# facebookresearch/fast3r

Hardware: NVIDIA H100
Metric: views_per_sec (higher is better)
Workload: dtype bf16

## Files before the change

fast3r_b200/csrc/common.cuh:

```cuda
#pragma once
#include <cuda.h>
#include <cuda_bf16.h>
#include <cuda_fp16.h>
#include <cuda_runtime.h>
#include <stdint.h>

#include <type_traits>

namespace f3r {

#define F3R_DEVICE __device__ __forceinline__

F3R_DEVICE uint32_t smem_u32(const void* p) { return static_cast<uint32_t>(__cvta_generic_to_shared(p)); }

F3R_DEVICE uint32_t lane_id() { return threadIdx.x & 31; }

F3R_DEVICE bool elect_one() {
  uint32_t pred = 0;
  asm volatile(
      "{\n\t.reg .pred P;\n\t"
      "elect.sync _|P, 0xffffffff;\n\t"
      "selp.u32 %0, 1, 0, P;\n\t}\n"
      : "=r"(pred));
  return pred != 0;
}

F3R_DEVICE void mbar_init(uint64_t* bar, uint32_t count) {
  asm volatile("mbarrier.init.shared::cta.b64 [%0], %1;" ::"r"(smem_u32(bar)), "r"(count));
}
F3R_DEVICE void fence_barrier_init() { asm volatile("fence.mbarrier_init.release.cluster;" ::: "memory"); }
F3R_DEVICE void fence_proxy_async_smem() { asm volatile("fence.proxy.async.shared::cta;" ::: "memory"); }

F3R_DEVICE void mbar_arrive(uint64_t* bar) {
  asm volatile("mbarrier.arrive.shared::cta.b64 _, [%0];" ::"r"(smem_u32(bar)) : "memory");
}
F3R_DEVICE void mbar_arrive_expect_tx(uint64_t* bar, uint32_t bytes) {
  asm volatile("mbarrier.arrive.expect_tx.shared::cta.b64 _, [%0], %1;" ::"r"(smem_u32(bar)), "r"(bytes) : "memory");
}
F3R_DEVICE bool mbar_try_wait(uint64_t* bar, uint32_t parity) {
  uint32_t ok;
  asm volatile(
      "{\n\t.reg .pred P;\n\t"
      "mbarrier.try_wait.parity.shared::cta.b64 P, [%1], %2;\n\t"
      "selp.u32 %0, 1, 0, P;\n\t}\n"
      : "=r"(ok)
      : "r"(smem_u32(bar)), "r"(parity)
      : "memory");
  return ok != 0;
}
F3R_DEVICE void mbar_wait(uint64_t* bar, uint32_t parity) {
  while (!mbar_try_wait(bar, parity)) {
  }
}

F3R_DEVICE void mbar_wait_relaxed(uint64_t* bar, uint32_t parity) {
  while (!mbar_try_wait(bar, parity)) asm volatile("nanosleep.u32 64;");
}

F3R_DEVICE void tma_prefetch_desc(const CUtensorMap* m) {
  asm volatile("prefetch.tensormap [%0];" ::"l"(reinterpret_cast<uint64_t>(m)) : "memory");
}
F3R_DEVICE void tma_load_2d(void* dst, const CUtensorMap* m, uint64_t* bar, int c0, int c1) {
  asm volatile(
      "cp.async.bulk.tensor.2d.shared::cluster.global.mbarrier::complete_tx::bytes [%0], [%1, {%3, %4}], [%2];"
      ::"r"(smem_u32(dst)), "l"(reinterpret_cast<uint64_t>(m)), "r"(smem_u32(bar)), "r"(c0), "r"(c1)
      : "memory");
}
F3R_DEVICE void tma_load_3d(void* dst, const CUtensorMap* m, uint64_t* bar, int c0, int c1, int c2) {
  asm volatile(
      "cp.async.bulk.tensor.3d.shared::cluster.global.mbarrier::complete_tx::bytes [%0], [%1, {%3, %4, %5}], [%2];"
      ::"r"(smem_u32(dst)), "l"(reinterpret_cast<uint64_t>(m)), "r"(smem_u32(bar)), "r"(c0), "r"(c1), "r"(c2)
      : "memory");
}
F3R_DEVICE void tma_load_4d(void* dst, const CUtensorMap* m, uint64_t* bar, int c0, int c1, int c2, int c3) {
  asm volatile(
      "cp.async.bulk.tensor.4d.shared::cluster.global.mbarrier::complete_tx::bytes [%0], [%1, {%3, %4, %5, %6}], [%2];"
      ::"r"(smem_u32(dst)), "l"(reinterpret_cast<uint64_t>(m)), "r"(smem_u32(bar)), "r"(c0), "r"(c1), "r"(c2),
      "r"(c3)
      : "memory");
}

F3R_DEVICE void tma_store_4d(const CUtensorMap* m, const void* src, int c0, int c1, int c2, int c3) {
  asm volatile("cp.async.bulk.tensor.4d.global.shared::cta.bulk_group [%0, {%2, %3, %4, %5}], [%1];"
               ::"l"(reinterpret_cast<uint64_t>(m)), "r"(smem_u32(src)), "r"(c0), "r"(c1), "r"(c2), "r"(c3)
               : "memory");
}
F3R_DEVICE void tma_reduce_add_4d(const CUtensorMap* m, const void* src, int c0, int c1, int c2, int c3) {
  asm volatile("cp.reduce.async.bulk.tensor.4d.global.shared::cta.add.tile.bulk_group [%0, {%2, %3, %4, %5}], [%1];"
               ::"l"(reinterpret_cast<uint64_t>(m)), "r"(smem_u32(src)), "r"(c0), "r"(c1), "r"(c2), "r"(c3)
               : "memory");
}
F3R_DEVICE void tma_store_commit() { asm volatile("cp.async.bulk.commit_group;" ::: "memory"); }
F3R_DEVICE void tma_store_wait_read() { asm volatile("cp.async.bulk.wait_group.read 0;" ::: "memory"); }
F3R_DEVICE void tma_store_wait_all() { asm volatile("cp.async.bulk.wait_group 0;" ::: "memory"); }

F3R_DEVICE void pdl_wait() { asm volatile("griddepcontrol.wait;" ::: "memory"); }
F3R_DEVICE void pdl_launch_dependents() { asm volatile("griddepcontrol.launch_dependents;" ::: "memory"); }

F3R_DEVICE uint32_t cluster_ctarank() { uint32_t r; asm volatile("mov.u32 %0, %%cluster_ctarank;" : "=r"(r)); return r; }
F3R_DEVICE uint32_t cluster_id_x() { uint32_t r; asm volatile("mov.u32 %0, %%clusterid.x;" : "=r"(r)); return r; }
F3R_DEVICE uint32_t num_clusters_x() { uint32_t r; asm volatile("mov.u32 %0, %%nclusterid.x;" : "=r"(r)); return r; }
F3R_DEVICE void cluster_sync_all() {
  asm volatile("barrier.cluster.arrive.release.aligned;" ::: "memory");
  asm volatile("barrier.cluster.wait.acquire.aligned;" ::: "memory");
}

F3R_DEVICE uint64_t make_smem_desc_sw128(uint32_t smem_addr) {
  uint64_t d = 0;
  d |= static_cast<uint64_t>((smem_addr & 0x3FFFF) >> 4);
  d |= static_cast<uint64_t>(1) << 16;
  d |= static_cast<uint64_t>(1024 >> 4) << 32;
  d |= static_cast<uint64_t>(1) << 62;
  return d;
}
F3R_DEVICE void wgmma_fence() { asm volatile("wgmma.fence.sync.aligned;" ::: "memory"); }
F3R_DEVICE void wgmma_commit() { asm volatile("wgmma.commit_group.sync.aligned;" ::: "memory"); }
template <int kPending>
F3R_DEVICE void wgmma_wait() { asm volatile("wgmma.wait_group.sync.aligned %0;" ::"n"(kPending) : "memory"); }
template <int kN>
F3R_DEVICE void fence_regs(float (&d)[kN]) {
#pragma unroll
  for (int i = 0; i < kN; ++i) asm volatile("" : "+f"(d[i])::"memory");
}


template <typename T>
constexpr bool is_f16 = std::is_same<T, __half>::value;

#define F3R_WGMMA_SS_N128(TY) \
  asm volatile( \
      "{\n\t.reg .pred p;\n\t" \
      "setp.ne.b32 p, %66, 0;\n\t" \
      "wgmma.mma_async.sync.aligned.m64n128k16.f32." TY "." TY " {%0, %1, %2, %3, %4, %5, %6, %7, %8, %9, %10, %11, %12, %13, %14, %15, %16, %17, %18, %19, %20, %21, %22, %23, %24, %25, %26, %27, %28, %29, %30, %31, %32, %33, %34, %35, %36, %37, %38, %39, %40, %41, %42, %43, %44, %45, %46, %47, %48, %49, %50, %51, %52, %53, %54, %55, %56, %57, %58, %59, %60, %61, %62, %63}, %64, %65, p, 1, 1, 0, %67;\n\t}\n" \
      : "+f"(d[0]), "+f"(d[1]), "+f"(d[2]), "+f"(d[3]), "+f"(d[4]), "+f"(d[5]), "+f"(d[6]), "+f"(d[7]), "+f"(d[8]), "+f"(d[9]), "+f"(d[10]), "+f"(d[11]), "+f"(d[12]), "+f"(d[13]), "+f"(d[14]), "+f"(d[15]), "+f"(d[16]), "+f"(d[17]), "+f"(d[18]), "+f"(d[19]), "+f"(d[20]), "+f"(d[21]), "+f"(d[22]), "+f"(d[23]), "+f"(d[24]), "+f"(d[25]), "+f"(d[26]), "+f"(d[27]), "+f"(d[28]), "+f"(d[29]), "+f"(d[30]), "+f"(d[31]), "+f"(d[32]), "+f"(d[33]), "+f"(d[34]), "+f"(d[35]), "+f"(d[36]), "+f"(d[37]), "+f"(d[38]), "+f"(d[39]), "+f"(d[40]), "+f"(d[41]), "+f"(d[42]), "+f"(d[43]), "+f"(d[44]), "+f"(d[45]), "+f"(d[46]), "+f"(d[47]), "+f"(d[48]), "+f"(d[49]), "+f"(d[50]), "+f"(d[51]), "+f"(d[52]), "+f"(d[53]), "+f"(d[54]), "+f"(d[55]), "+f"(d[56]), "+f"(d[57]), "+f"(d[58]), "+f"(d[59]), "+f"(d[60]), "+f"(d[61]), "+f"(d[62]), "+f"(d[63]) \
      : "l"(a_desc), "l"(b_desc), "r"(accumulate), "n"(kTransB))
template <int kTransB, typename T = __nv_bfloat16>
F3R_DEVICE void wgmma_ss_n128(float (&d)[64], uint64_t a_desc, uint64_t b_desc, uint32_t accumulate) {
  if constexpr (is_f16<T>) F3R_WGMMA_SS_N128("f16");
  else F3R_WGMMA_SS_N128("bf16");
}

#define F3R_WGMMA_SS_N256(TY) \
  asm volatile( \
      "{\n\t.reg .pred p;\n\t" \
      "setp.ne.b32 p, %130, 0;\n\t" \
      "wgmma.mma_async.sync.aligned.m64n256k16.f32." TY "." TY " {%0, %1, %2, %3, %4, %5, %6, %7, %8, %9, %10, %11, %12, %13, %14, %15, %16, %17, %18, %19, %20, %21, %22, %23, %24, %25, %26, %27, %28, %29, %30, %31, %32, %33, %34, %35, %36, %37, %38, %39, %40, %41, %42, %43, %44, %45, %46, %47, %48, %49, %50, %51, %52, %53, %54, %55, %56, %57, %58, %59, %60, %61, %62, %63, %64, %65, %66, %67, %68, %69, %70, %71, %72, %73, %74, %75, %76, %77, %78, %79, %80, %81, %82, %83, %84, %85, %86, %87, %88, %89, %90, %91, %92, %93, %94, %95, %96, %97, %98, %99, %100, %101, %102, %103, %104, %105, %106, %107, %108, %109, %110, %111, %112, %113, %114, %115, %116, %117, %118, %119, %120, %121, %122, %123, %124, %125, %126, %127}, %128, %129, p, 1, 1, 0, %131;\n\t}\n" \
      : "+f"(d[0]), "+f"(d[1]), "+f"(d[2]), "+f"(d[3]), "+f"(d[4]), "+f"(d[5]), "+f"(d[6]), "+f"(d[7]), "+f"(d[8]), "+f"(d[9]), "+f"(d[10]), "+f"(d[11]), "+f"(d[12]), "+f"(d[13]), "+f"(d[14]), "+f"(d[15]), "+f"(d[16]), "+f"(d[17]), "+f"(d[18]), "+f"(d[19]), "+f"(d[20]), "+f"(d[21]), "+f"(d[22]), "+f"(d[23]), "+f"(d[24]), "+f"(d[25]), "+f"(d[26]), "+f"(d[27]), "+f"(d[28]), "+f"(d[29]), "+f"(d[30]), "+f"(d[31]), "+f"(d[32]), "+f"(d[33]), "+f"(d[34]), "+f"(d[35]), "+f"(d[36]), "+f"(d[37]), "+f"(d[38]), "+f"(d[39]), "+f"(d[40]), "+f"(d[41]), "+f"(d[42]), "+f"(d[43]), "+f"(d[44]), "+f"(d[45]), "+f"(d[46]), "+f"(d[47]), "+f"(d[48]), "+f"(d[49]), "+f"(d[50]), "+f"(d[51]), "+f"(d[52]), "+f"(d[53]), "+f"(d[54]), "+f"(d[55]), "+f"(d[56]), "+f"(d[57]), "+f"(d[58]), "+f"(d[59]), "+f"(d[60]), "+f"(d[61]), "+f"(d[62]), "+f"(d[63]), "+f"(d[64]), "+f"(d[65]), "+f"(d[66]), "+f"(d[67]), "+f"(d[68]), "+f"(d[69]), "+f"(d[70]), "+f"(d[71]), "+f"(d[72]), "+f"(d[73]), "+f"(d[74]), "+f"(d[75]), "+f"(d[76]), "+f"(d[77]), "+f"(d[78]), "+f"(d[79]), "+f"(d[80]), "+f"(d[81]), "+f"(d[82]), "+f"(d[83]), "+f"(d[84]), "+f"(d[85]), "+f"(d[86]), "+f"(d[87]), "+f"(d[88]), "+f"(d[89]), "+f"(d[90]), "+f"(d[91]), "+f"(d[92]), "+f"(d[93]), "+f"(d[94]), "+f"(d[95]), "+f"(d[96]), "+f"(d[97]), "+f"(d[98]), "+f"(d[99]), "+f"(d[100]), "+f"(d[101]), "+f"(d[102]), "+f"(d[103]), "+f"(d[104]), "+f"(d[105]), "+f"(d[106]), "+f"(d[107]), "+f"(d[108]), "+f"(d[109]), "+f"(d[110]), "+f"(d[111]), "+f"(d[112]), "+f"(d[113]), "+f"(d[114]), "+f"(d[115]), "+f"(d[116]), "+f"(d[117]), "+f"(d[118]), "+f"(d[119]), "+f"(d[120]), "+f"(d[121]), "+f"(d[122]), "+f"(d[123]), "+f"(d[124]), "+f"(d[125]), "+f"(d[126]), "+f"(d[127]) \
      : "l"(a_desc), "l"(b_desc), "r"(accumulate), "n"(kTransB))
template <int kTransB, typename T = __nv_bfloat16>
F3R_DEVICE void wgmma_ss_n256(float (&d)[128], uint64_t a_desc, uint64_t b_desc, uint32_t accumulate) {
  if constexpr (is_f16<T>) F3R_WGMMA_SS_N256("f16");
  else F3R_WGMMA_SS_N256("bf16");
}

#define F3R_WGMMA_RS_N64(TY) \
  asm volatile( \
      "{\n\t.reg .pred p;\n\t" \
      "setp.ne.b32 p, %37, 0;\n\t" \
      "wgmma.mma_async.sync.aligned.m64n64k16.f32." TY "." TY " {%0, %1, %2, %3, %4, %5, %6, %7, %8, %9, %10, %11, %12, %13, %14, %15, %16, %17, %18, %19, %20, %21, %22, %23, %24, %25, %26, %27, %28, %29, %30, %31}, {%32, %33, %34, %35}, %36, p, 1, 1, %38;\n\t}\n" \
      : "+f"(d[0]), "+f"(d[1]), "+f"(d[2]), "+f"(d[3]), "+f"(d[4]), "+f"(d[5]), "+f"(d[6]), "+f"(d[7]), "+f"(d[8]), "+f"(d[9]), "+f"(d[10]), "+f"(d[11]), "+f"(d[12]), "+f"(d[13]), "+f"(d[14]), "+f"(d[15]), "+f"(d[16]), "+f"(d[17]), "+f"(d[18]), "+f"(d[19]), "+f"(d[20]), "+f"(d[21]), "+f"(d[22]), "+f"(d[23]), "+f"(d[24]), "+f"(d[25]), "+f"(d[26]), "+f"(d[27]), "+f"(d[28]), "+f"(d[29]), "+f"(d[30]), "+f"(d[31]) \
      : "r"(a[0]), "r"(a[1]), "r"(a[2]), "r"(a[3]), "l"(b_desc), "r"(accumulate), "n"(kTransB))
template <int kTransB, typename T = __nv_bfloat16>
F3R_DEVICE void wgmma_rs_n64(float (&d)[32], const uint32_t (&a)[4], uint64_t b_desc, uint32_t accumulate) {
  if constexpr (is_f16<T>) F3R_WGMMA_RS_N64("f16");
  else F3R_WGMMA_RS_N64("bf16");
}

F3R_DEVICE uint32_t pack_bf16(float lo, float hi) {
  __nv_bfloat162 v = __floats2bfloat162_rn(lo, hi);
  return *reinterpret_cast<uint32_t*>(&v);
}
F3R_DEVICE float bf16_lo(uint32_t v) { return __uint_as_float(v << 16); }
F3R_DEVICE float bf16_hi(uint32_t v) { return __uint_as_float(v & 0xFFFF0000u); }
F3R_DEVICE uint32_t pack_f16(float lo, float hi) {
  __half2 v = __floats2half2_rn(lo, hi);
  return *reinterpret_cast<uint32_t*>(&v);
}
F3R_DEVICE float f16_lo(uint32_t v) { return __half2float(__ushort_as_half(static_cast<unsigned short>(v & 0xFFFFu))); }
F3R_DEVICE float f16_hi(uint32_t v) { return __half2float(__ushort_as_half(static_cast<unsigned short>(v >> 16))); }

template <typename T>
struct Half16 {
  static F3R_DEVICE uint32_t pack(float lo, float hi) { return pack_bf16(lo, hi); }
  static F3R_DEVICE float lo(uint32_t v) { return bf16_lo(v); }
  static F3R_DEVICE float hi(uint32_t v) { return bf16_hi(v); }
};
template <>
struct Half16<__half> {
  static F3R_DEVICE uint32_t pack(float lo, float hi) { return pack_f16(lo, hi); }
  static F3R_DEVICE float lo(uint32_t v) { return f16_lo(v); }
  static F3R_DEVICE float hi(uint32_t v) { return f16_hi(v); }
};
F3R_DEVICE float gelu_erf(float x) { return 0.5f * x * (1.0f + erff(x * 0.70710678118654752440f)); }

}
```

fast3r_b200/csrc/gemm.cu:

```cuda
#include "common.cuh"
#include "f3r_kernels.h"

namespace f3r {

constexpr int BLOCK_M = 128;
constexpr int BLOCK_K = 64;
constexpr int GEMM_THREADS = 384;
constexpr int XCH_STRIDE = 68;

template <int BLOCK_N>
struct GemmCfg {
  static constexpr int kStages = (BLOCK_N == 256) ? 3 : 4;
  static constexpr int kABytes = BLOCK_M * BLOCK_K * 2;
  static constexpr int kBBytes = BLOCK_N * BLOCK_K * 2;
  static constexpr int kStageBytes = kABytes + kBBytes;
  static constexpr int kXchBytes = 64 * XCH_STRIDE * 4;
  static constexpr int kSmemBytes =
      kStages * kStageBytes + 1024  + 1024  + 8 * 4096  + 2 * kXchBytes;
};

struct ResChunk {
  uint4 r0[8];
  uint2 r1[8];
};

__device__ __forceinline__ size_t out_offset(const GemmArgs& p, int m, int col0, int img, int py, int px) {
  if (p.epi == EPI_CONVT) {
    const int ij = col0 / p.ct_cout, o0 = col0 % p.ct_cout, k = p.ct_k;
    const int oy = py * k + ij / k, ox = px * k + ij % k;
    return ((static_cast<size_t>(img) * p.H * k + oy) * (p.W * k) + ox) * p.ct_cout + o0;
  }
  return static_cast<size_t>(m) * p.ldo + col0;
}

__device__ __forceinline__ void prefetch_res(const GemmArgs& p, ResChunk& rc, size_t off_row, bool ok_row, int lane) {
  if (p.res0 == nullptr && p.res1 == nullptr) return;
  const unsigned okmask = __ballot_sync(0xffffffffu, ok_row);
#pragma unroll
  for (int i = 0; i < 8; ++i) {
    const int rr = 4 * i + (lane >> 3);
    const size_t off = __shfl_sync(0xffffffffu, off_row, rr) + (lane & 7) * 4;
    if (!((okmask >> rr) & 1)) continue;
    if (p.res0 != nullptr) {
      if (p.res0_f32) rc.r0[i] = *reinterpret_cast<const uint4*>(static_cast<const float*>(p.res0) + off);
      else {
        const uint2 t = *reinterpret_cast<const uint2*>(static_cast<const uint16_t*>(p.res0) + off);
        rc.r0[i].x = t.x; rc.r0[i].y = t.y;
      }
    }
    if (p.res1 != nullptr) rc.r1[i] = *reinterpret_cast<const uint2*>(static_cast<const uint16_t*>(p.res1) + off);
  }
}

__device__ __forceinline__ void gelu_fast(float& x) {
  const float z = __fmul_rn(fabsf(x), 0.70710678118654752440f);
  const float u = fmaf(z, 0.3275911f, 1.0f);
  float t;
  asm("rcp.approx.ftz.f32 %0, %1;" : "=f"(t) : "f"(u));
  float q = fmaf(t, 1.061405429f, -1.453152027f);
  q = fmaf(q, t, 1.421413741f);
  q = fmaf(q, t, -0.284496736f);
  q = fmaf(q, t, 0.254829592f);
  q = __fmul_rn(q, t);
  const float a = __fmul_rn(__fmul_rn(z, z), -1.4426950408889634f);
  float e;
  asm("ex2.approx.ftz.f32 %0, %1;" : "=f"(e) : "f"(a));
  const float r = copysignf(fmaf(q, -e, 1.0f), x);
  const float h = __fmul_rn(x, 0.5f);
  x = fmaf(h, r, h);
}
__device__ __forceinline__ bool epilogue_rows(const GemmArgs& p, float (&v)[32], int m, int col0, bool row_ok,
                                              float (&fin)[4], bool add_bias, const float* w4s) {
  if (p.bias != nullptr && add_bias) {
    const float4* b4 = reinterpret_cast<const float4*>(p.bias + (p.epi == EPI_CONVT ? (col0 % p.ct_cout) : col0));
#pragma unroll
    for (int i = 0; i < 8; ++i) {
      float4 b = __ldg(b4 + i);
      v[4 * i + 0] += b.x; v[4 * i + 1] += b.y; v[4 * i + 2] += b.z; v[4 * i + 3] += b.w;
    }
  }
  if (p.epi == EPI_ROPE && col0 < p.rope_cols && row_ok) {
    const int t = m % p.tok_per_img;
    const int pos = ((col0 >> 5) & 1) ? (t % p.grid_w) : (t / p.grid_w);
    const float4* c4 = reinterpret_cast<const float4*>(p.rope_cos + pos * 16);
    const float4* s4 = reinterpret_cast<const float4*>(p.rope_sin + pos * 16);
#pragma unroll
    for (int i = 0; i < 4; ++i) {
      float4 c = __ldg(c4 + i), s = __ldg(s4 + i);
      float cc[4] = {c.x, c.y, c.z, c.w}, ss[4] = {s.x, s.y, s.z, s.w};
#pragma unroll
      for (int e = 0; e < 4; ++e) {
        const int j = 4 * i + e;
        const float a = v[j], b = v[j + 16];
        v[j] = a * cc[e] - b * ss[e];
        v[j + 16] = b * cc[e] + a * ss[e];
      }
    }
  }
  if (p.epi == EPI_IDXEMB && row_ok) {
    const int id = __ldg(p.emb_ids + (p.tok_per_img > 0 ? m / p.tok_per_img : m));
    const float4* e4 = reinterpret_cast<const float4*>(p.emb_table + static_cast<size_t>(id) * p.N + col0);
#pragma unroll
    for (int i = 0; i < 8; ++i) {
      float4 e = __ldg(e4 + i);
      v[4 * i + 0] += e.x; v[4 * i + 1] += e.y; v[4 * i + 2] += e.z; v[4 * i + 3] += e.w;
    }
  }
  if (p.epi == EPI_FINAL) {
    if (row_ok) {
#pragma unroll
      for (int o = 0; o < 4; ++o) {
        const float4* w = reinterpret_cast<const float4*>(w4s + o * p.N + col0);
        float acc = fin[o];
#pragma unroll
        for (int i = 0; i < 8; ++i) {
          const float4 ww = w[i];
          acc = fmaf(fmaxf(v[4 * i + 0], 0.f), ww.x, acc);
          acc = fmaf(fmaxf(v[4 * i + 1], 0.f), ww.y, acc);
          acc = fmaf(fmaxf(v[4 * i + 2], 0.f), ww.z, acc);
          acc = fmaf(fmaxf(v[4 * i + 3], 0.f), ww.w, acc);
        }
        fin[o] = acc;
      }
    }
    return false;
  }
  return true;
}

template <typename T>
__device__ __forceinline__ void epilogue_store(const GemmArgs& p, const float (&v)[32], const ResChunk& rc, uint8_t* stage,
                                               int lane, int m, int col0, size_t off_row, bool ok_row) {
  using H = Half16<T>;
#pragma unroll
  for (int j = 0; j < 8; ++j)
    *reinterpret_cast<float4*>(stage + lane * 128 + ((j ^ (lane & 7)) << 4)) =
        make_float4(v[4 * j], v[4 * j + 1], v[4 * j + 2], v[4 * j + 3]);
  __syncwarp();
  const unsigned okmask = __ballot_sync(0xffffffffu, ok_row);
  const int cj = lane & 7;
  const bool to_b = p.split_col > 0 && col0 >= p.split_col;
#pragma unroll
  for (int i = 0; i < 8; ++i) {
    const int rr = 4 * i + (lane >> 3);
    const size_t off = __shfl_sync(0xffffffffu, off_row, rr) + cj * 4;
    const int mrow = __shfl_sync(0xffffffffu, m, rr);
    if (!((okmask >> rr) & 1)) continue;
    const float4 a = *reinterpret_cast<const float4*>(stage + rr * 128 + ((cj ^ (rr & 7)) << 4));
    float x0 = a.x, x1 = a.y, x2 = a.z, x3 = a.w;
    if (p.res0 != nullptr) {
      if (p.res0_f32) {
        x0 += __uint_as_float(rc.r0[i].x); x1 += __uint_as_float(rc.r0[i].y);
        x2 += __uint_as_float(rc.r0[i].z); x3 += __uint_as_float(rc.r0[i].w);
      } else {
        x0 += H::lo(rc.r0[i].x); x1 += H::hi(rc.r0[i].x); x2 += H::lo(rc.r0[i].y); x3 += H::hi(rc.r0[i].y);
      }
    }
    if (p.res1 != nullptr) {
      x0 += H::lo(rc.r1[i].x); x1 += H::hi(rc.r1[i].x); x2 += H::lo(rc.r1[i].y); x3 += H::hi(rc.r1[i].y);
    }
    if (p.out1 != nullptr) {
      uint2 o;
      o.x = H::pack(fmaxf(x0, 0.f), fmaxf(x1, 0.f));
      o.y = H::pack(fmaxf(x2, 0.f), fmaxf(x3, 0.f));
      *reinterpret_cast<uint2*>(static_cast<T*>(p.out1) + off) = o;
    }
    if (p.out0 == nullptr) continue;
    if (p.act == ACT_RELU) {
      x0 = fmaxf(x0, 0.f); x1 = fmaxf(x1, 0.f); x2 = fmaxf(x2, 0.f); x3 = fmaxf(x3, 0.f);
    } else if (p.act == ACT_GELU) {
      gelu_fast(x0); gelu_fast(x1); gelu_fast(x2); gelu_fast(x3);
    }
    void* base = p.out0;
    size_t o = off;
    if (to_b) {
      base = p.out0b;
      o = static_cast<size_t>(mrow) * p.ldo_b + (col0 - p.split_col) + cj * 4;
    }
    if (p.out0_f32) {
      *reinterpret_cast<float4*>(static_cast<float*>(base) + o) = make_float4(x0, x1, x2, x3);
    } else {
      uint2 q;
      q.x = H::pack(x0, x1);
      q.y = H::pack(x2, x3);
      *reinterpret_cast<uint2*>(static_cast<T*>(base) + o) = q;
    }
  }
  __syncwarp();
}

template <typename T>
__device__ __forceinline__ void epilogue_tma(const GemmArgs& p, float (&v)[32], uint8_t* stage, int lane,
                                             const CUtensorMap* map, bool reduce, int c_col, int c_x, int c_y, int c_img) {
  if (p.act == ACT_RELU) {
#pragma unroll
    for (int i = 0; i < 32; ++i) v[i] = fmaxf(v[i], 0.f);
  } else if (p.act == ACT_GELU) {
#pragma unroll
    for (int i = 0; i < 32; ++i) gelu_fast(v[i]);
  }
  if (lane == 0) tma_store_wait_read();
  __syncwarp();
  if (p.out0_f32) {
#pragma unroll
    for (int j = 0; j < 8; ++j)
      *reinterpret_cast<float4*>(stage + lane * 128 + ((j ^ (lane & 7)) << 4)) =
          make_float4(v[4 * j], v[4 * j + 1], v[4 * j + 2], v[4 * j + 3]);
  } else {
#pragma unroll
    for (int j = 0; j < 4; ++j) {
      uint4 q;
      q.x = Half16<T>::pack(v[8 * j + 0], v[8 * j + 1]);
      q.y = Half16<T>::pack(v[8 * j + 2], v[8 * j + 3]);
      q.z = Half16<T>::pack(v[8 * j + 4], v[8 * j + 5]);
      q.w = Half16<T>::pack(v[8 * j + 6], v[8 * j + 7]);
      *reinterpret_cast<uint4*>(stage + lane * 64 + ((j ^ ((lane >> 1) & 3)) << 4)) = q;
    }
  }
  fence_proxy_async_smem();
  __syncwarp();
  if (lane == 0) {
    if (reduce) tma_reduce_add_4d(map, stage, c_col, c_x, c_y, c_img);
    else tma_store_4d(map, stage, c_col, c_x, c_y, c_img);
    tma_store_commit();
  }
}

template <int BLOCK_N, typename T>
__global__ void __launch_bounds__(GEMM_THREADS, 1)
gemm_kernel(const __grid_constant__ CUtensorMap tmap_a, const __grid_constant__ CUtensorMap tmap_b,
            const __grid_constant__ CUtensorMap tmap_o0, const __grid_constant__ CUtensorMap tmap_o0b,
            const __grid_constant__ GemmArgs p) {
  using Cfg = GemmCfg<BLOCK_N>;
  extern __shared__ uint8_t smem_raw[];
  uint8_t* smem = reinterpret_cast<uint8_t*>((reinterpret_cast<uintptr_t>(smem_raw) + 1023) & ~uintptr_t(1023));
  uint8_t* smem_a = smem;
  uint8_t* smem_b = smem + Cfg::kStages * Cfg::kABytes;
  uint64_t* bars = reinterpret_cast<uint64_t*>(smem + Cfg::kStages * Cfg::kStageBytes);
  uint64_t* full_bar = bars;
  uint64_t* empty_bar = bars + Cfg::kStages;
  uint8_t* stage_base = smem + Cfg::kStages * Cfg::kStageBytes + 1024;
  float* fin_smem = reinterpret_cast<float*>(stage_base);
  float* w4_smem = reinterpret_cast<float*>(stage_base + 4096);
  float* xch_base = reinterpret_cast<float*>(stage_base + 8 * 4096);

  const int warp = threadIdx.x >> 5;
  const int lane = threadIdx.x & 31;

  if (threadIdx.x == 0) {
    tma_prefetch_desc(&tmap_a);
    tma_prefetch_desc(&tmap_b);
    for (int s = 0; s < Cfg::kStages; ++s) { mbar_init(&full_bar[s], 1); mbar_init(&empty_bar[s], 2); }
    fence_barrier_init();
  }
  if (p.epi == EPI_FINAL)
    for (int i = threadIdx.x; i < 4 * p.N; i += GEMM_THREADS) w4_smem[i] = __ldg(p.w4 + i);
  __syncthreads();
  pdl_wait();
  pdl_launch_dependents();

  const int num_out_tiles = p.num_m_tiles * p.num_n_tiles;
  const int num_tiles = num_out_tiles * p.k_split;
  const int k_chunks = (p.K + BLOCK_K - 1) / BLOCK_K;
  const int k_iters = p.taps * k_chunks;

  if (warp < 4) {
    asm volatile("setmaxnreg.dec.sync.aligned.u32 40;");
    if (warp == 0 && lane == 0) {
      int stage = 0; uint32_t phase = 0;
      for (int item = blockIdx.x; item < num_tiles; item += gridDim.x) {
        const int tile = item % num_out_tiles, ks = item / num_out_tiles;
        const int it0 = ks * k_iters / p.k_split, it1 = (ks + 1) * k_iters / p.k_split;
        const int mt = tile / p.num_n_tiles, nt = tile % p.num_n_tiles;
        const int tx = mt % p.tiles_x, ty = (mt / p.tiles_x) % p.tiles_y, img = mt / (p.tiles_x * p.tiles_y);
        const int x0 = tx * p.bw, y0 = ty * p.bh, n0 = nt * BLOCK_N;
        for (int it = it0; it < it1; ++it) {
          const int tap = it / k_chunks, kc = it % k_chunks;
          int dy = 0, dx = 0;
          if (p.taps == 9) { dy = tap / 3 - 1; dx = tap % 3 - 1; }
          mbar_wait_relaxed(&empty_bar[stage], phase ^ 1);
          mbar_arrive_expect_tx(&full_bar[stage], Cfg::kStageBytes);
          tma_load_4d(smem_a + stage * Cfg::kABytes, &tmap_a, &full_bar[stage], kc * BLOCK_K, x0 + dx, y0 + dy, img);
          tma_load_3d(smem_b + stage * Cfg::kBBytes, &tmap_b, &full_bar[stage], kc * BLOCK_K, tap, n0);
          if (++stage == Cfg::kStages) { stage = 0; phase ^= 1; }
        }
      }
    }
  } else {
    asm volatile("setmaxnreg.inc.sync.aligned.u32 232;");
    const int cg = (warp - 4) >> 2;
    const int wg_warp = warp & 3;
    const int wg_tid = threadIdx.x & 127;
    const int half = wg_warp >> 1;
    const int r_loc = (wg_warp & 1) * 32 + lane;
    const int r = cg * 64 + r_loc;
    float* xch = xch_base + cg * 64 * XCH_STRIDE;
    uint8_t* stage_buf = stage_base + (warp - 4) * 4096;
    const int bar_id = 1 + cg;
    constexpr int kAcc = BLOCK_N / 2;
    int stage = 0; uint32_t phase = 0;
    for (int item = blockIdx.x; item < num_tiles; item += gridDim.x) {
      const int tile = item % num_out_tiles, ks = item / num_out_tiles;
      const int it0 = ks * k_iters / p.k_split, it1 = (ks + 1) * k_iters / p.k_split;
      const bool add_bias = ks == 0;
      float acc[kAcc];
#pragma unroll
      for (int i = 0; i < kAcc; ++i) acc[i] = 0.f;
      int prev = -1;
      for (int it = it0; it < it1; ++it) {
        mbar_wait(&full_bar[stage], phase);
        const uint64_t a_desc = make_smem_desc_sw128(smem_u32(smem_a + stage * Cfg::kABytes + cg * 64 * 128));
        const uint64_t b_desc = make_smem_desc_sw128(smem_u32(smem_b + stage * Cfg::kBBytes));
        fence_regs(acc);
        wgmma_fence();
#pragma unroll
        for (int k = 0; k < BLOCK_K / 16; ++k) {
          if constexpr (BLOCK_N == 256) wgmma_ss_n256<0, T>(acc, a_desc + 2 * k, b_desc + 2 * k, 1u);
          else wgmma_ss_n128<0, T>(acc, a_desc + 2 * k, b_desc + 2 * k, 1u);
        }
        wgmma_commit();
        wgmma_wait<1>();
        fence_regs(acc);
        if (prev >= 0 && wg_tid == 0) mbar_arrive(&empty_bar[prev]);
        prev = stage;
        if (++stage == Cfg::kStages) { stage = 0; phase ^= 1; }
      }
      wgmma_wait<0>();
      fence_regs(acc);
      if (prev >= 0 && wg_tid == 0) mbar_arrive(&empty_bar[prev]);

      const int mt = tile / p.num_n_tiles, nt = tile % p.num_n_tiles;
      const int tx = mt % p.tiles_x, ty = (mt / p.tiles_x) % p.tiles_y, img = mt / (p.tiles_x * p.tiles_y);
      const int px = tx * p.bw + r % p.bw, py = ty * p.bh + r / p.bw;
      const bool row_ok = (px < p.W) && (py < p.H) && (mt < p.num_m_tiles);
      const int m = (img * p.H + py) * p.W + px;
      const int n_valid = min(BLOCK_N / 32, (p.N - nt * BLOCK_N + 31) / 32);
      float fin[4] = {0.f, 0.f, 0.f, 0.f};
#pragma unroll
      for (int cp = 0; cp < BLOCK_N / 64; ++cp) {
        asm volatile("bar.sync %0, 128;" ::"r"(bar_id) : "memory");
        {
          const int fr = wg_warp * 16 + (lane >> 2), fc = 2 * (lane & 3);
#pragma unroll
          for (int j = 0; j < 8; ++j) {
            const int jj = cp * 8 + j;
            *reinterpret_cast<float2*>(xch + fr * XCH_STRIDE + 8 * j + fc) = make_float2(acc[4 * jj], acc[4 * jj + 1]);
            *reinterpret_cast<float2*>(xch + (fr + 8) * XCH_STRIDE + 8 * j + fc) =
                make_float2(acc[4 * jj + 2], acc[4 * jj + 3]);
          }
        }
        asm volatile("bar.sync %0, 128;" ::"r"(bar_id) : "memory");
        const int c = 2 * cp + half;
        if (c >= n_valid) continue;
        const int col0 = nt * BLOCK_N + c * 32;
        float v[32];
#pragma unroll
        for (int i = 0; i < 8; ++i) {
          const float4 t = *reinterpret_cast<const float4*>(xch + r_loc * XCH_STRIDE + half * 32 + 4 * i);
          v[4 * i] = t.x; v[4 * i + 1] = t.y; v[4 * i + 2] = t.z; v[4 * i + 3] = t.w;
        }
        if (epilogue_rows(p, v, m, col0, row_ok, fin, add_bias, w4_smem) && !(p.debug & 1)) {
          if (p.tma_epi) {
            const bool to_b = p.split_col > 0 && col0 >= p.split_col;
            const int r0 = cg * 64 + (wg_warp & 1) * 32;
            epilogue_tma<T>(p, v, stage_buf, lane, to_b ? &tmap_o0b : &tmap_o0, p.tma_epi == 2,
                         to_b ? col0 - p.split_col : col0, tx * p.bw + (r0 & (p.bw - 1)), ty * p.bh + (r0 >> p.bw_log2),
                         mt < p.num_m_tiles ? img : p.NB);
          } else {
            const size_t off = out_offset(p, m, col0, img, py, px);
            ResChunk rc;
            prefetch_res(p, rc, off, row_ok, lane);
            epilogue_store<T>(p, v, rc, stage_buf, lane, m, col0, off, row_ok);
          }
        }
      }
      if (p.epi == EPI_FINAL) {
        float* slot = fin_smem + r * 4;
        if (half == 1) { slot[0] = fin[0]; slot[1] = fin[1]; slot[2] = fin[2]; slot[3] = fin[3]; }
        asm volatile("bar.sync %0, 128;" ::"r"(bar_id) : "memory");
        if (half == 0 && row_ok) {
          const float x = fin[0] + slot[0] + __ldg(p.b4 + 0), y = fin[1] + slot[1] + __ldg(p.b4 + 1);
          const float z = fin[2] + slot[2] + __ldg(p.b4 + 2), c = fin[3] + slot[3] + __ldg(p.b4 + 3);
          const float d = sqrtf(x * x + y * y + z * z);
          const float sc = expm1f(d) / fmaxf(d, 1e-8f);
          float* pt = p.pts + static_cast<size_t>(m) * 3;
          pt[0] = x * sc; pt[1] = y * sc; pt[2] = z * sc;
          p.conf[m] = 1.f + expf(c);
        }
      }
    }
    if (p.tma_epi && lane == 0) tma_store_wait_all();
  }
}

template <int BLOCK_N, typename T>
static cudaError_t launch_gemm_t(const CUtensorMap& ta, const CUtensorMap& tb, const CUtensorMap& to0,
                                 const CUtensorMap& to0b, const GemmArgs& a, int num_sms, cudaStream_t stream) {
  const int items = a.num_m_tiles * a.num_n_tiles * a.k_split;
  return launch(gemm_kernel<BLOCK_N, T>, items < num_sms ? items : num_sms, GEMM_THREADS, GemmCfg<BLOCK_N>::kSmemBytes,
                stream, true, ta, tb, to0, to0b, a);
}

cudaError_t launch_gemm(int block_n, int f16, const CUtensorMap& ta, const CUtensorMap& tb, const CUtensorMap& to0,
                        const CUtensorMap& to0b, const GemmArgs& a, int num_sms, cudaStream_t stream) {
  if (f16) {
    if (block_n == 256) return launch_gemm_t<256, __half>(ta, tb, to0, to0b, a, num_sms, stream);
    return launch_gemm_t<128, __half>(ta, tb, to0, to0b, a, num_sms, stream);
  }
  if (block_n == 256) return launch_gemm_t<256, __nv_bfloat16>(ta, tb, to0, to0b, a, num_sms, stream);
  return launch_gemm_t<128, __nv_bfloat16>(ta, tb, to0, to0b, a, num_sms, stream);
}

}
```

Before: 152.0.

## Write TMA-epilogue output directly from wgmma fragments into swizzled smem slabs

For the TMA epilogue path, skips the fp32 exchange-buffer transpose and writes accumulator fragments straight into swizzled per-warpgroup output slabs. Bias, RoPE, index embedding and activation are applied in registers, and the activation is specialized at compile time. TMA stores for a whole tile are issued in bulk, and fp32 output double-buffers the slabs with partial wait_group. The intent is to remove the extra shared-memory round trip and several barrier pairs per column chunk. The cost is a duplicated epilogue logic path that could diverge from epilogue_rows semantics, for example residual handling and any epilogue variant not reimplemented here.

```diff
diff --git a/fast3r_b200/csrc/common.cuh b/fast3r_b200/csrc/common.cuh
--- a/fast3r_b200/csrc/common.cuh
+++ b/fast3r_b200/csrc/common.cuh
@@ -91,7 +91,8 @@
                : "memory");
 }
 F3R_DEVICE void tma_store_commit() { asm volatile("cp.async.bulk.commit_group;" ::: "memory"); }
-F3R_DEVICE void tma_store_wait_read() { asm volatile("cp.async.bulk.wait_group.read 0;" ::: "memory"); }
+template <int kPending>
+F3R_DEVICE void tma_store_wait_read() { asm volatile("cp.async.bulk.wait_group.read %0;" ::"n"(kPending) : "memory"); }
 F3R_DEVICE void tma_store_wait_all() { asm volatile("cp.async.bulk.wait_group 0;" ::: "memory"); }
 
 F3R_DEVICE void pdl_wait() { asm volatile("griddepcontrol.wait;" ::: "memory"); }
diff --git a/fast3r_b200/csrc/gemm.cu b/fast3r_b200/csrc/gemm.cu
--- a/fast3r_b200/csrc/gemm.cu
+++ b/fast3r_b200/csrc/gemm.cu
@@ -7,6 +7,7 @@
 constexpr int BLOCK_K = 64;
 constexpr int GEMM_THREADS = 384;
 constexpr int XCH_STRIDE = 68;
+constexpr int kSlabBytes = 32768;
 
 template <int BLOCK_N>
 struct GemmCfg {
@@ -15,8 +16,9 @@
   static constexpr int kBBytes = BLOCK_N * BLOCK_K * 2;
   static constexpr int kStageBytes = kABytes + kBBytes;
   static constexpr int kXchBytes = 64 * XCH_STRIDE * 4;
-  static constexpr int kSmemBytes =
-      kStages * kStageBytes + 1024  + 1024  + 8 * 4096  + 2 * kXchBytes;
+  static constexpr int kEpiBytes = 8 * 4096 + 2 * kXchBytes;
+  static_assert(2 * kSlabBytes <= kEpiBytes, "output slabs exceed the epilogue region");
+  static constexpr int kSmemBytes = kStages * kStageBytes + 1024  + 1024  + kEpiBytes;
 };
 
 struct ResChunk {
@@ -189,40 +191,150 @@
   __syncwarp();
 }
 
-template <typename T>
-__device__ __forceinline__ void epilogue_tma(const GemmArgs& p, float (&v)[32], uint8_t* stage, int lane,
-                                             const CUtensorMap* map, bool reduce, int c_col, int c_x, int c_y, int c_img) {
-  if (p.act == ACT_RELU) {
-#pragma unroll
-    for (int i = 0; i < 32; ++i) v[i] = fmaxf(v[i], 0.f);
-  } else if (p.act == ACT_GELU) {
-#pragma unroll
-    for (int i = 0; i < 32; ++i) gelu_fast(v[i]);
-  }
-  if (lane == 0) tma_store_wait_read();
-  __syncwarp();
-  if (p.out0_f32) {
-#pragma unroll
-    for (int j = 0; j < 8; ++j)
-      *reinterpret_cast<float4*>(stage + lane * 128 + ((j ^ (lane & 7)) << 4)) =
-          make_float4(v[4 * j], v[4 * j + 1], v[4 * j + 2], v[4 * j + 3]);
-  } else {
-#pragma unroll
-    for (int j = 0; j < 4; ++j) {
-      uint4 q;
-      q.x = Half16<T>::pack(v[8 * j + 0], v[8 * j + 1]);
-      q.y = Half16<T>::pack(v[8 * j + 2], v[8 * j + 3]);
-      q.z = Half16<T>::pack(v[8 * j + 4], v[8 * j + 5]);
-      q.w = Half16<T>::pack(v[8 * j + 6], v[8 * j + 7]);
-      *reinterpret_cast<uint4*>(stage + lane * 64 + ((j ^ ((lane >> 1) & 3)) << 4)) = q;
-    }
-  }
-  fence_proxy_async_smem();
-  __syncwarp();
-  if (lane == 0) {
-    if (reduce) tma_reduce_add_4d(map, stage, c_col, c_x, c_y, c_img);
-    else tma_store_4d(map, stage, c_col, c_x, c_y, c_img);
-    tma_store_commit();
+__device__ __forceinline__ void wg_bar_sync(int bar_id) { asm volatile("bar.sync %0, 128;" ::"r"(bar_id) : "memory"); }
+
+template <int BLOCK_N, typename T, bool F32, int ACT>
+__device__ __forceinline__ void epilogue_frag(const GemmArgs& p, float (&acc)[BLOCK_N / 2], uint8_t* slab,
+                                              const CUtensorMap* map0, const CUtensorMap* map0b, int cg, int wg_warp,
+                                              int lane, int bar_id, int mt, int nt, int tx, int ty, int img,
+                                              bool add_bias) {
+  using H = Half16<T>;
+  constexpr bool f32 = F32;
+  const bool issuer = lane == 0;
+  const int n_valid = min(BLOCK_N / 32, (p.N - nt * BLOCK_N + 31) / 32);
+  const int q = lane & 3;
+  const int hbox = wg_warp >> 1;
+  const int rb = (wg_warp & 1) * 16 + (lane >> 2);
+  const bool has_bias = p.bias != nullptr && add_bias;
+  int key[2];
+#pragma unroll
+  for (int hr = 0; hr < 2; ++hr) {
+    const int r = cg * 64 + hbox * 32 + rb + 8 * hr;
+    const int px = tx * p.bw + r % p.bw, py = ty * p.bh + r / p.bw;
+    const int m = (img * p.H + py) * p.W + px;
+    key[hr] = -1;
+    if ((px < p.W) && (py < p.H) && (mt < p.num_m_tiles)) {
+      key[hr] = 0;
+      if (p.epi == EPI_ROPE) {
+        const int t = m % p.tok_per_img;
+        key[hr] = (t / p.grid_w) | ((t % p.grid_w) << 16);
+      } else if (p.epi == EPI_IDXEMB) {
+        key[hr] = __ldg(p.emb_ids + (p.tok_per_img > 0 ? m / p.tok_per_img : m));
+      }
+    }
+  }
+#pragma unroll
+  for (int cp = 0; cp < BLOCK_N / 64; ++cp) {
+    uint8_t* buf = f32 ? slab + (cp & 1) * 16384 : slab;
+    float2 bias2[2][4];
+#pragma unroll
+    for (int ch = 0; ch < 2; ++ch)
+#pragma unroll
+      for (int g = 0; g < 4; ++g)
+        bias2[ch][g] = (has_bias && 2 * cp + ch < n_valid)
+                           ? __ldg(reinterpret_cast<const float2*>(p.bias + nt * BLOCK_N + (2 * cp + ch) * 32 + 8 * g + 2 * q))
+                           : make_float2(0.f, 0.f);
+    if (cp == 0 || f32) {
+      if (issuer) {
+        if (f32) tma_store_wait_read<1>();
+        else tma_store_wait_read<0>();
+      }
+      wg_bar_sync(bar_id);
+    }
+#pragma unroll
+    for (int ch = 0; ch < 2; ++ch) {
+      const int c = 2 * cp + ch;
+      if (c >= n_valid) continue;
+      const int col0 = nt * BLOCK_N + c * 32;
+      if (has_bias) {
+#pragma unroll
+        for (int g = 0; g < 4; ++g) {
+          const float2 b = bias2[ch][g];
+          acc[16 * c + 4 * g + 0] += b.x; acc[16 * c + 4 * g + 1] += b.y;
+          acc[16 * c + 4 * g + 2] += b.x; acc[16 * c + 4 * g + 3] += b.y;
+        }
+      }
+      if (p.epi == EPI_ROPE && col0 < p.rope_cols) {
+#pragma unroll
+        for (int hr = 0; hr < 2; ++hr) {
+          if (key[hr] < 0) continue;
+          const int pos = ((col0 >> 5) & 1) ? (key[hr] >> 16) : (key[hr] & 0xffff);
+#pragma unroll
+          for (int g = 0; g < 2; ++g) {
+            const float2 c2 = __ldg(reinterpret_cast<const float2*>(p.rope_cos + pos * 16 + 8 * g + 2 * q));
+            const float2 s2 = __ldg(reinterpret_cast<const float2*>(p.rope_sin + pos * 16 + 8 * g + 2 * q));
+            const float cc[2] = {c2.x, c2.y}, ss[2] = {s2.x, s2.y};
+#pragma unroll
+            for (int e = 0; e < 2; ++e) {
+              float& va = acc[16 * c + 4 * g + 2 * hr + e];
+              float& vb = acc[16 * c + 4 * (g + 2) + 2 * hr + e];
+              const float a = va, b = vb;
+              va = a * cc[e] - b * ss[e];
+              vb = b * cc[e] + a * ss[e];
+            }
+          }
+        }
+      }
+      if (p.epi == EPI_IDXEMB) {
+#pragma unroll
+        for (int hr = 0; hr < 2; ++hr) {
+          if (key[hr] < 0) continue;
+          const float* e_row = p.emb_table + static_cast<size_t>(key[hr]) * p.N + col0;
+#pragma unroll
+          for (int g = 0; g < 4; ++g) {
+            const float2 e = __ldg(reinterpret_cast<const float2*>(e_row + 8 * g + 2 * q));
+            acc[16 * c + 4 * g + 2 * hr] += e.x; acc[16 * c + 4 * g + 2 * hr + 1] += e.y;
+          }
+        }
+      }
+      if constexpr (ACT == ACT_RELU) {
+#pragma unroll
+        for (int i = 0; i < 16; ++i) acc[16 * c + i] = fmaxf(acc[16 * c + i], 0.f);
+      } else if constexpr (ACT == ACT_GELU) {
+#pragma unroll
+        for (int i = 0; i < 16; ++i) gelu_fast(acc[16 * c + i]);
+      }
+      if (f32) {
+        uint8_t* box = buf + (ch * 2 + hbox) * 4096;
+#pragma unroll
+        for (int g = 0; g < 4; ++g)
+#pragma unroll
+          for (int hr = 0; hr < 2; ++hr) {
+            const int row = rb + 8 * hr, k = 2 * g + (q >> 1);
+            *reinterpret_cast<float2*>(box + row * 128 + ((k ^ (row & 7)) << 4) + 8 * (q & 1)) =
+                make_float2(acc[16 * c + 4 * g + 2 * hr], acc[16 * c + 4 * g + 2 * hr + 1]);
+          }
+      } else {
+        uint8_t* box = slab + (c * 2 + hbox) * 2048;
+#pragma unroll
+        for (int g = 0; g < 4; ++g)
+#pragma unroll
+          for (int hr = 0; hr < 2; ++hr) {
+            const int row = rb + 8 * hr;
+            *reinterpret_cast<uint32_t*>(box + row * 64 + ((g ^ ((row >> 1) & 3)) << 4) + 4 * q) =
+                H::pack(acc[16 * c + 4 * g + 2 * hr], acc[16 * c + 4 * g + 2 * hr + 1]);
+          }
+      }
+    }
+    if (f32 || cp == BLOCK_N / 64 - 1) {
+      fence_proxy_async_smem();
+      wg_bar_sync(bar_id);
+      if (issuer) {
+        for (int b = wg_warp; b < (f32 ? 4 : BLOCK_N / 16); b += 4) {
+          const int c = (f32 ? 2 * cp : 0) + (b >> 1), h = b & 1;
+          if (c >= n_valid) break;
+          const int col0 = nt * BLOCK_N + c * 32;
+          const bool to_b = p.split_col > 0 && col0 >= p.split_col;
+          const int r0 = cg * 64 + h * 32;
+          const uint8_t* src = f32 ? buf + ((c & 1) * 2 + h) * 4096 : slab + (c * 2 + h) * 2048;
+          const int c_x = tx * p.bw + (r0 & (p.bw - 1)), c_y = ty * p.bh + (r0 >> p.bw_log2);
+          const int c_img = mt < p.num_m_tiles ? img : p.NB;
+          if (p.tma_epi == 2) tma_reduce_add_4d(map0, src, col0, c_x, c_y, c_img);
+          else tma_store_4d(to_b ? map0b : map0, src, to_b ? col0 - p.split_col : col0, c_x, c_y, c_img);
+        }
+        tma_store_commit();
+      }
+    }
   }
 }
 
@@ -331,6 +443,25 @@
 
       const int mt = tile / p.num_n_tiles, nt = tile % p.num_n_tiles;
       const int tx = mt % p.tiles_x, ty = (mt / p.tiles_x) % p.tiles_y, img = mt / (p.tiles_x * p.tiles_y);
+      if (p.tma_epi) {
+        if (!(p.debug & 1)) {
+          uint8_t* slab = stage_base + cg * kSlabBytes;
+#define F3R_EPI_FRAG(F32, ACT)                                                                                         \
+  epilogue_frag<BLOCK_N, T, F32, ACT>(p, acc, slab, &tmap_o0, &tmap_o0b, cg, wg_warp, lane, bar_id, mt, nt, tx, ty, img, \
+                                      add_bias)
+          if (p.out0_f32) {
+            if (p.act == ACT_GELU) F3R_EPI_FRAG(true, ACT_GELU);
+            else if (p.act == ACT_RELU) F3R_EPI_FRAG(true, ACT_RELU);
+            else F3R_EPI_FRAG(true, ACT_NONE);
+          } else {
+            if (p.act == ACT_GELU) F3R_EPI_FRAG(false, ACT_GELU);
+            else if (p.act == ACT_RELU) F3R_EPI_FRAG(false, ACT_RELU);
+            else F3R_EPI_FRAG(false, ACT_NONE);
+          }
+#undef F3R_EPI_FRAG
+        }
+        continue;
+      }
       const int px = tx * p.bw + r % p.bw, py = ty * p.bh + r / p.bw;
       const bool row_ok = (px < p.W) && (py < p.H) && (mt < p.num_m_tiles);
       const int m = (img * p.H + py) * p.W + px;
@@ -360,18 +491,10 @@
           v[4 * i] = t.x; v[4 * i + 1] = t.y; v[4 * i + 2] = t.z; v[4 * i + 3] = t.w;
         }
         if (epilogue_rows(p, v, m, col0, row_ok, fin, add_bias, w4_smem) && !(p.debug & 1)) {
-          if (p.tma_epi) {
-            const bool to_b = p.split_col > 0 && col0 >= p.split_col;
-            const int r0 = cg * 64 + (wg_warp & 1) * 32;
-            epilogue_tma<T>(p, v, stage_buf, lane, to_b ? &tmap_o0b : &tmap_o0, p.tma_epi == 2,
-                         to_b ? col0 - p.split_col : col0, tx * p.bw + (r0 & (p.bw - 1)), ty * p.bh + (r0 >> p.bw_log2),
-                         mt < p.num_m_tiles ? img : p.NB);
-          } else {
-            const size_t off = out_offset(p, m, col0, img, py, px);
-            ResChunk rc;
-            prefetch_res(p, rc, off, row_ok, lane);
-            epilogue_store<T>(p, v, rc, stage_buf, lane, m, col0, off, row_ok);
-          }
+          const size_t off = out_offset(p, m, col0, img, py, px);
+          ResChunk rc;
+          prefetch_res(p, rc, off, row_ok, lane);
+          epilogue_store<T>(p, v, rc, stage_buf, lane, m, col0, off, row_ok);
         }
       }
       if (p.epi == EPI_FINAL) {
```

Result: faster. 154.4, median of 6 (+1.6%).
